# liuzuxin/FSRL

Hardware: NVIDIA H100
Metric: env-steps/sec (collect+update) SafetyCarCircle-v0 PPO-Lag (higher is better)
Workload: dtype f32

## Files before the change

### fsrl_b200/csrc/ppo_persist.cu

```cuda
#include "ppo_persist.cuh"
#include "arena.cuh"
#include "ppo_loss.cuh"
#include "wgmma.cuh"
#include <cuda_pipeline.h>
#include <cstdlib>
#include <cmath>
#include <vector>

namespace fsrl {
namespace pp {

using namespace wg;

constexpr int WQ = 2;
constexpr int NEPI = 128 * WQ;
constexpr int TPB = NEPI + 32;
constexpr int C1 = 16 / WQ;
constexpr int C2 = 32 / WQ;
constexpr int RB = 64;
constexpr int MB = 256;
constexpr int KC = 32, NCH = 256 / KC;
constexpr int SLOT_BYTES = 32768, NSLOT = 4;
constexpr int A_CHUNK = 64 * KC * 4;
constexpr int ACC_LD = 68;
constexpr int OUTP = 8;
constexpr int H_ = 256;
constexpr int IMG = 65536;
enum { I_H1A_HI, I_H1A_LO, I_H1T_HI, I_H1T_LO, I_DZA_HI, I_DZA_LO, I_DZT_HI, I_DZT_LO, I_W2A_HI, I_W2A_LO, I_W2B_HI, I_W2B_LO, N_IMG };
constexpr int DB2P_OFF = N_IMG * IMG;
constexpr int DW3P_OFF = DB2P_OFF + 4 * H_;
constexpr int DB3P_OFF = DW3P_OFF + 4 * H_ * OUTP;
constexpr int MAXD = 40;
constexpr int XS_OFF = 2 * SLOT_BYTES;
static_assert(XS_OFF >= 2 * 32 * 65 * 2 * 4 && XS_OFF >= 2 * (MAXD + 1) * 64 * 4 &&
              XS_OFF + 128 * (MAXD + 1) * 4 <= NSLOT * SLOT_BYTES, "staged rows overlap the ring's scratch or dW1 partials");
constexpr int NSMAX = (MAXD + 1) * 32 + 32 + 32 * OUTP + 16;
constexpr int SLICE_OFF = DB3P_OFF + 4 * 16;
constexpr int NET_WS = SLICE_OFF + 8 * NSMAX;
constexpr int SUMSQ_FLOATS = 128;
constexpr int FLAG_LINE = 32;
constexpr int F_A = 0, F_C = 1, F_PER_NET = 2;
constexpr int TILE_PK = (64 * 64 / NEPI + 2) / 3;
constexpr int TILE_FLOATS = TILE_PK * NEPI * 4;
constexpr int SLICE_PK = (NSMAX + 2) / 3;
constexpr int XG_PER_NET = 16 * TILE_FLOATS + 8 * SLICE_PK * 4;
constexpr int MAX_MB = 16384;
constexpr long long WAIT_CYCLES = 6000000000LL;

struct Args {
    fsrl_ppo_update_t u;
    int n_mb, slot0;
    long long adam_t0;
    float* ws;
    unsigned* flags;
    int* err;
    const float* adam_tab;
    long long* dbg;
    int dbg_step;
    unsigned dp_seq;
    int dp_direct;
};
constexpr int DBG_CH = 48;
constexpr int DBG_N = DBG_CH + 2 * 3 * NCH;
#define STAMP(i) do { if (P.dbg && t == P.dbg_step) P.dbg[(size_t)blockIdx.x * DBG_N + (i)] = clock64(); } while (0)

struct AdamS { float w1, b2, w2, rbc2s, eps, neg_step; };
__device__ __forceinline__ float adam_one(float p, float g, float& m, float& v, const AdamS& a) {
    m = m + a.w1 * (g - m);
    v = v * a.b2 + (a.w2 * g) * g;
    const float sq = v > 0.f ? v * rsqrtf(v) : 0.f;
    const float denom = fmaf(sq, a.rbc2s, a.eps);
    return p + __fdividef(a.neg_step * m, denom);
}

__device__ __forceinline__ void fail(int* err, int code) {
    *reinterpret_cast<volatile int*>(err) = code;
    __threadfence_system();
    asm volatile("trap;");
}
__device__ __forceinline__ uint32_t pk_hash(float x, float y, float z) {
    const uint32_t a = __float_as_uint(x), b = __float_as_uint(y), c = __float_as_uint(z);
    return a ^ __funnelshift_l(b, b, 11) ^ __funnelshift_l(c, c, 22);
}
__device__ __forceinline__ bool pk_ok(const float4& v, uint32_t tag) { return (__float_as_uint(v.w) ^ pk_hash(v.x, v.y, v.z)) == tag; }
__device__ __forceinline__ void st_packet(float* p, float x, float y, float z, uint32_t tag) {
    asm volatile("st.relaxed.sys.global.v4.f32 [%0], {%1,%2,%3,%4};" ::"l"(p), "f"(x), "f"(y), "f"(z), "f"(__uint_as_float(tag ^ pk_hash(x, y, z))) : "memory");
}
__device__ __forceinline__ float4 ld_packet(const float* p) {
    float4 v;
    asm volatile("ld.relaxed.sys.global.v4.f32 {%0,%1,%2,%3}, [%4];" : "=f"(v.x), "=f"(v.y), "=f"(v.z), "=f"(v.w) : "l"(p) : "memory");
    return v;
}

__device__ __noinline__ float3 dp_gather(const float* src, long long stride, int me, int world, uint32_t tag,
                                        float ox, float oy, float oz, int* err, int code) {
    const long long t0w = clock64();
    float ax = 0.f, ay = 0.f, az = 0.f;
    for (int r0 = 0; r0 < world; r0 += 4) {
        float4 v[4];
        bool ok;
        do {
            ok = true;
#pragma unroll
            for (int k = 0; k < 4; ++k)
                if (r0 + k < world && r0 + k != me) v[k] = ld_packet(src + (size_t)(r0 + k) * stride);
#pragma unroll
            for (int k = 0; k < 4; ++k)
                if (r0 + k < world && r0 + k != me) ok = ok && pk_ok(v[k], tag);
            if (!ok && clock64() - t0w > 4 * WAIT_CYCLES) fail(err, code);
        } while (!ok);
#pragma unroll
        for (int k = 0; k < 4; ++k) {
            if (r0 + k >= world) continue;
            if (r0 + k == me) { ax += ox; ay += oy; az += oz; }
            else { ax += v[k].x; ay += v[k].y; az += v[k].z; }
        }
    }
    return make_float3(ax, ay, az);
}
__device__ __noinline__ void dp_push_all(const float* const* xg, size_t off, int me, int world, float x, float y, float z, uint32_t tag) {
    for (int r = 0; r < world; ++r)
        if (r != me) st_packet(const_cast<float*>(xg[r]) + off, x, y, z, tag);
}

__device__ __forceinline__ uint32_t mapa_u32(uint32_t local_saddr, uint32_t rank) {
    uint32_t r;
    asm volatile("mapa.shared::cluster.u32 %0, %1, %2;" : "=r"(r) : "r"(local_saddr), "r"(rank));
    return r;
}
__device__ __forceinline__ void st_cluster4(uint32_t raddr, float4 v) {
    asm volatile("st.shared::cluster.v4.f32 [%0], {%1,%2,%3,%4};" ::"r"(raddr), "f"(v.x), "f"(v.y), "f"(v.z), "f"(v.w) : "memory");
}
__device__ __forceinline__ void st_async4(uint32_t raddr, float4 v, uint32_t rbar) {
    asm volatile("st.async.weak.shared::cluster.mbarrier::complete_tx::bytes.v4.f32 [%0], {%1,%2,%3,%4}, [%5];"
                 ::"r"(raddr), "f"(v.x), "f"(v.y), "f"(v.z), "f"(v.w), "r"(rbar) : "memory");
}
__device__ __forceinline__ float ld_cluster(uint32_t raddr) {
    float v;
    asm volatile("ld.shared::cluster.f32 %0, [%1];" : "=f"(v) : "r"(raddr) : "memory");
    return v;
}
__device__ __forceinline__ void mbar_arrive_release_cluster2(uint32_t raddr0, uint32_t raddr1) {
    asm volatile("fence.acq_rel.cluster;\n\t"
                 "mbarrier.arrive.relaxed.cluster.shared::cluster.b64 _, [%0];\n\t"
                 "mbarrier.arrive.relaxed.cluster.shared::cluster.b64 _, [%1];" ::"r"(raddr0), "r"(raddr1) : "memory");
}
__device__ __forceinline__ bool mbar_wait_cluster(uint64_t* bar, uint32_t parity, long long timeout_cycles) {
    const long long t0 = clock64();
    while (true) {
        uint32_t ok;
        asm volatile(
            "{\n\t.reg .pred p;\n\t"
            "mbarrier.try_wait.parity.acquire.cluster.shared::cta.b64 p, [%1], %2;\n\t"
            "selp.u32 %0, 1, 0, p;\n\t}"
            : "=r"(ok) : "r"(smem_u32(bar)), "r"(parity) : "memory");
        if (ok) return true;
        if (clock64() - t0 > timeout_cycles) return false;
    }
}
__device__ __forceinline__ void cluster_sync_all() {
    asm volatile("barrier.cluster.arrive.release.aligned;\n\tbarrier.cluster.wait.acquire.aligned;" ::: "memory");
}

__device__ __forceinline__ bool elect_one() {
    uint32_t pred = 0;
    asm volatile(
        "{\n\t.reg .b32 rx;\n\t.reg .pred px;\n\t"
        "elect.sync rx|px, 0xffffffff;\n\t"
        "selp.u32 %0, 1, 0, px;\n\t}"
        : "=r"(pred));
    return pred != 0;
}
__device__ __forceinline__ void epi_bar() { asm volatile("bar.sync 1, %0;" ::"n"(NEPI) : "memory"); }
__device__ __forceinline__ void prefetch_l2(const void* p) { asm volatile("prefetch.global.L2 [%0];" ::"l"(p)); }

template <int NC>
__device__ __forceinline__ void acc_ld(const float* accs, int row, int col, float (&v)[NC]) {
#pragma unroll
    for (int q = 0; q < NC / 4; ++q) {
        const float4 x = *reinterpret_cast<const float4*>(accs + row * ACC_LD + col + 4 * q);
        v[4 * q] = x.x; v[4 * q + 1] = x.y; v[4 * q + 2] = x.z; v[4 * q + 3] = x.w;
    }
}
template <int NC>
__device__ __forceinline__ void acc_st(float* accs, int row, int col, const float (&v)[NC]) {
#pragma unroll
    for (int q = 0; q < NC / 4; ++q)
        *reinterpret_cast<float4*>(accs + row * ACC_LD + col + 4 * q) = make_float4(v[4 * q], v[4 * q + 1], v[4 * q + 2], v[4 * q + 3]);
}

template <int N>
__device__ __forceinline__ void gemm_phase(const unsigned char* ring, unsigned& qq, uint64_t* bar_full, uint32_t empty_r,
                                           float (&dm)[N / 2], float (&dc)[N / 2], int* err, int code, int lane,
                                           const Args& P, int t, int g) {
#pragma unroll
    for (int e = 0; e < N / 2; ++e) dm[e] = dc[e] = 0.f;
    const uint32_t ring_a = smem_u32(ring);
    constexpr uint32_t b_lbo = 16 * N, b_chunk = N * KC * 4;
    for (int j = 0; j < NCH; ++j, ++qq) {
        const int s = qq % NSLOT;
        if (!mbar_wait(&bar_full[s], (qq / NSLOT) & 1, WAIT_CYCLES)) fail(err, code);
#ifdef FSRL_PPO_CHUNK_STAMPS
        if (P.dbg && t == P.dbg_step && threadIdx.x < 32) P.dbg[(size_t)blockIdx.x * DBG_N + DBG_CH + 3 * NCH * g + 2 * NCH + j] = clock64();
#endif
        __syncwarp();
        wgmma_fence();
        const uint32_t base = ring_a + (uint32_t)s * SLOT_BYTES;
        const uint64_t ah0 = smem_desc(base, 1024, 128), al0 = smem_desc(base + A_CHUNK, 1024, 128);
        const uint64_t bh0 = smem_desc(base + 2 * A_CHUNK, b_lbo, 128), bl0 = smem_desc(base + 2 * A_CHUNK + b_chunk, b_lbo, 128);
#pragma unroll
        for (int ks = 0; ks < KC / 8; ++ks) {
            const uint64_t ah = ah0 + ks * (2048 / 16), al = al0 + ks * (2048 / 16);
            const uint64_t bh = bh0 + ks * (2 * b_lbo / 16), bl = bl0 + ks * (2 * b_lbo / 16);
            if constexpr (N == 32) {
                mma_m64n32k8_tf32(dc, al, bh);
                mma_m64n32k8_tf32(dc, ah, bl);
                mma_m64n32k8_tf32(dm, ah, bh);
            } else {
                mma_m64n64k8_tf32(dc, al, bh);
                mma_m64n64k8_tf32(dc, ah, bl);
                mma_m64n64k8_tf32(dm, ah, bh);
            }
        }
        wgmma_commit();
        if (j > 0) {
            wgmma_wait<1>();
            __syncwarp();
            if (lane < 8) mbar_arrive_cluster(empty_r + 8 * ((qq - 1) % NSLOT));
        }
    }
    wgmma_wait<0>();
    reg_fence(dm); reg_fence(dc);
    __syncwarp();
    if (lane < 8) mbar_arrive_cluster(empty_r + 8 * ((qq - 1) % NSLOT));
}
template <int N>
__device__ __forceinline__ void stage_acc(float* accs, const float (&dm)[N / 2], const float (&dc)[N / 2], int wq, int sp,
                                          int lane) {
    if (wq == 0) {
        const int r = 16 * sp + (lane >> 2);
#pragma unroll
        for (int i = 0; i < N / 8; ++i) {
            const int c = 8 * i + 2 * (lane & 3);
            *reinterpret_cast<float2*>(accs + r * ACC_LD + c) = make_float2(dm[4 * i] + dc[4 * i], dm[4 * i + 1] + dc[4 * i + 1]);
            *reinterpret_cast<float2*>(accs + (r + 8) * ACC_LD + c) =
                make_float2(dm[4 * i + 2] + dc[4 * i + 2], dm[4 * i + 3] + dc[4 * i + 3]);
        }
    }
    asm volatile("bar.sync %0, 64;" ::"r"(2 + sp) : "memory");
}

__device__ __forceinline__ void copy_operand(unsigned char* dst, const float* src, uint32_t bytes, uint64_t* bar, int g, int i,
                                             uint16_t cta_mask) {
    if (g == 1) {
        bulk_g2s(dst, src, bytes, bar);
        bulk_g2s(dst + bytes, src + IMG, bytes, bar);
        return;
    }
    const uint32_t piece = 2 * bytes / g, off = i * piece, part = off / bytes, in = off % bytes;
    bulk_g2s_multicast(dst + off, src + (size_t)part * IMG + in / 4, piece, bar, cta_mask);
}

template <int NC, int W>
__device__ __forceinline__ void transposed_stage(float* scr, const float (&hi)[NC], const float (&lo)[NC], int row, int c0) {
    constexpr int LO = W * 65;
#pragma unroll
    for (int j = 0; j < NC; ++j) {
        scr[(c0 + j) * 65 + row] = hi[j];
        scr[LO + (c0 + j) * 65 + row] = lo[j];
    }
}
template <int W>
__device__ __forceinline__ void transposed_flush(const float* scr, int et, float* img_hi, int row_base, int col_base) {
    constexpr int LO = W * 65;
    const int col = et % W;
    constexpr int GPT = 16 / (NEPI / W);
    const int g0 = (et / W) * GPT;
    float* dst = img_hi + (size_t)(row_base >> 2) * 256 + (size_t)(col_base + col) * 4;
#pragma unroll
    for (int q = 0; q < GPT; ++q) {
        const int g = g0 + q;
        const float* sh = scr + col * 65 + 4 * g;
        *reinterpret_cast<float4*>(dst + (size_t)g * 256) = make_float4(sh[0], sh[1], sh[2], sh[3]);
        *reinterpret_cast<float4*>(dst + IMG + (size_t)g * 256) = make_float4(sh[LO], sh[LO + 1], sh[LO + 2], sh[LO + 3]);
    }
}
template <int NC, int W>
__device__ __forceinline__ void store_transposed(float* scr, const float (&hi)[NC], const float (&lo)[NC], int row, int c0,
                                                 int et, float* img_hi, int row_base, int col_base) {
    transposed_stage<NC, W>(scr, hi, lo, row, c0);
    epi_bar();
    transposed_flush<W>(scr, et, img_hi, row_base, col_base);
    epi_bar();
}

__device__ __forceinline__ void stage_rows(float* xs, const float* obs, long long row0, int a, int D, int et) {
    const int i = et >> 1;
    const float* src = obs + (row0 + 64 * a + i + (i & 64)) * D;
    float* dst = xs + i * (D | 1);
    for (int d = et & 1; d < D; d += 2) __pipeline_memcpy_async(dst + d, src + d, 4);
    __pipeline_commit();
}

__device__ __forceinline__ float half_sum(float v) {
#pragma unroll
    for (int o = 8; o > 0; o >>= 1) v += __shfl_xor_sync(0xffffffffu, v, o);
    return v;
}

struct SliceMap {
    int w1, b2, w3, b3, n;
    __device__ __host__ SliceMap(int D) { w1 = 0; b2 = (D + 1) * 32; w3 = b2 + 32; b3 = w3 + 32 * OUTP; n = b3 + 16; }
};

struct DpCtx {
    const float* const* xg;
    long long region;
    int me, world;
    uint32_t tag;
    int* err;
    int direct;
};
__device__ __forceinline__ int dp_owner(int et, int q, int world) { return (int)((unsigned)((et >> 5) * TILE_PK + q) % (unsigned)world); }

__device__ __noinline__ void dp_tile_send(DpCtx d, size_t off, const float* accs, int trow, int cb2, int et) {
    float g[C2];
    acc_ld<C2>(accs, trow, cb2, g);
#pragma unroll
    for (int q = 0; q < TILE_PK; ++q) {
        const size_t o_q = (size_t)d.me * d.region + off + (size_t)q * NEPI * 4;
        const float x = g[3 * q], y = 3 * q + 1 < C2 ? g[3 * q + 1] : 0.f, z = 3 * q + 2 < C2 ? g[3 * q + 2] : 0.f;
        if (d.direct) {
            dp_push_all(d.xg, o_q, d.me, d.world, x, y, z, d.tag);
        } else {
            const int o = dp_owner(et, q, d.world);
            if (o != d.me) st_packet(const_cast<float*>(d.xg[o]) + o_q, x, y, z, d.tag);
        }
    }
}
__device__ __noinline__ void dp_tile_reduce(DpCtx d, size_t off, float* accs, int trow, int cb2, int et) {
    float g[C2];
    acc_ld<C2>(accs, trow, cb2, g);
    const float inv_world = 1.0f / (float)d.world;
    const float* loc = d.xg[d.me];
#pragma unroll
    for (int q = 0; q < TILE_PK; ++q) {
        if (dp_owner(et, q, d.world) != d.me) continue;
        const float3 s3 = dp_gather(loc + off + (size_t)q * NEPI * 4, d.region, d.me, d.world, d.tag, g[3 * q],
                                    3 * q + 1 < C2 ? g[3 * q + 1] : 0.f, 3 * q + 2 < C2 ? g[3 * q + 2] : 0.f, d.err, 41);
        const float ax = s3.x * inv_world, ay = s3.y * inv_world, az = s3.z * inv_world;
        dp_push_all(d.xg, (size_t)FSRL_P2P_MAX_RANKS * d.region + off + (size_t)q * NEPI * 4, d.me, d.world, ax, ay, az, d.tag);
        g[3 * q] = ax;
        if (3 * q + 1 < C2) g[3 * q + 1] = ay;
        if (3 * q + 2 < C2) g[3 * q + 2] = az;
    }
    acc_st<C2>(accs, trow, cb2, g);
}
__device__ __noinline__ float dp_tile_finish(DpCtx d, size_t off, float* accs, int trow, int cb2, int et) {
    float g[C2];
    const long long t0w = clock64();
    if (d.direct) {
        float own[C2];
        acc_ld<C2>(accs, trow, cb2, own);
#pragma unroll
        for (int jq = 0; jq < C2; ++jq) g[jq] = 0.f;
        for (int r = 0; r < d.world; ++r) {
            if (r == d.me) {
#pragma unroll
                for (int jq = 0; jq < C2; ++jq) g[jq] += own[jq];
                continue;
            }
            const float* src = d.xg[d.me] + (size_t)r * d.region + off;
            float4 v[TILE_PK];
            bool ok;
            do {
                ok = true;
#pragma unroll
                for (int q = 0; q < TILE_PK; ++q) v[q] = ld_packet(src + (size_t)q * NEPI * 4);
#pragma unroll
                for (int q = 0; q < TILE_PK; ++q) ok = ok && pk_ok(v[q], d.tag);
                if (!ok && clock64() - t0w > 4 * WAIT_CYCLES) fail(d.err, 42);
            } while (!ok);
#pragma unroll
            for (int q = 0; q < TILE_PK; ++q) {
                g[3 * q] += v[q].x;
                if (3 * q + 1 < C2) g[3 * q + 1] += v[q].y;
                if (3 * q + 2 < C2) g[3 * q + 2] += v[q].z;
            }
        }
        const float inv_world = 1.0f / (float)d.world;
        float sq = 0.f;
#pragma unroll
        for (int jq = 0; jq < C2; ++jq) { g[jq] *= inv_world; sq = fmaf(g[jq], g[jq], sq); }
        acc_st<C2>(accs, trow, cb2, g);
        return sq;
    }
    const float* res = d.xg[d.me] + (size_t)FSRL_P2P_MAX_RANKS * d.region + off;
    acc_ld<C2>(accs, trow, cb2, g);
    float4 v[TILE_PK];
    bool ok;
    do {
        ok = true;
#pragma unroll
        for (int q = 0; q < TILE_PK; ++q)
            if (dp_owner(et, q, d.world) != d.me) v[q] = ld_packet(res + (size_t)q * NEPI * 4);
#pragma unroll
        for (int q = 0; q < TILE_PK; ++q)
            if (dp_owner(et, q, d.world) != d.me) ok = ok && pk_ok(v[q], d.tag);
        if (!ok && clock64() - t0w > 4 * WAIT_CYCLES) fail(d.err, 42);
    } while (!ok);
    float sq = 0.f;
#pragma unroll
    for (int q = 0; q < TILE_PK; ++q) {
        if (dp_owner(et, q, d.world) == d.me) continue;
        g[3 * q] = v[q].x;
        if (3 * q + 1 < C2) g[3 * q + 1] = v[q].y;
        if (3 * q + 2 < C2) g[3 * q + 2] = v[q].z;
    }
#pragma unroll
    for (int jq = 0; jq < C2; ++jq) sq = fmaf(g[jq], g[jq], sq);
    acc_st<C2>(accs, trow, cb2, g);
    return sq;
}
__device__ __noinline__ void dp_slices(DpCtx d, size_t off_s, float* sp_g, int n, int et) {
    const int n3 = (n + 2) / 3;
    const float inv_world = 1.0f / (float)d.world;
    for (int i = et; i < n3; i += NEPI)
        dp_push_all(d.xg, (size_t)d.me * d.region + off_s + 4 * (size_t)i, d.me, d.world,
                    sp_g[3 * i], 3 * i + 1 < n ? sp_g[3 * i + 1] : 0.f, 3 * i + 2 < n ? sp_g[3 * i + 2] : 0.f, d.tag);
    const float* loc = d.xg[d.me];
    for (int i = et; i < n3; i += NEPI) {
        const float3 s3 = dp_gather(loc + off_s + 4 * (size_t)i, d.region, d.me, d.world, d.tag, sp_g[3 * i],
                                    3 * i + 1 < n ? sp_g[3 * i + 1] : 0.f, 3 * i + 2 < n ? sp_g[3 * i + 2] : 0.f, d.err, 40);
        sp_g[3 * i] = s3.x * inv_world;
        if (3 * i + 1 < n) sp_g[3 * i + 1] = s3.y * inv_world;
        if (3 * i + 2 < n) sp_g[3 * i + 2] = s3.z * inv_world;
    }
}

__device__ __forceinline__ bool red_cta() { return ((blockIdx.x >> 3) & 3) == ((blockIdx.x & 7) >> 2); }

__device__ __noinline__ float dp_tail(DpCtx d, size_t off_t, size_t off_s, float* accs, float* sp_g, int n, int trow, int cb2,
                                      int et, bool tile, bool slice) {
    if (tile && !d.direct) dp_tile_reduce(d, off_t, accs, trow, cb2, et);
    if (slice) dp_slices(d, off_s, sp_g, n, et);
    __syncwarp();
    return tile ? dp_tile_finish(d, off_t, accs, trow, cb2, et) : 0.f;
}

template <bool DP>
__global__ void __launch_bounds__(TPB, 1) ppo_persist_kernel(const Args P) {
    extern __shared__ __align__(1024) unsigned char smem_raw[];
    __shared__ __align__(8) uint64_t bar_full[NSLOT], bar_empty[NSLOT], bar_b, bar_w1;
    __shared__ float s_red[4][320];
    __shared__ float s_misc[32];
    __shared__ AdamS s_adam;
    __shared__ const float* s_xg[2][FSRL_P2P_MAX_RANKS];
    const fsrl_ppo_update_t& u = P.u;
    const int tid = threadIdx.x, warp = tid >> 5, lane = tid & 31;
    const int net = blockIdx.x >> 5, c = blockIdx.x & 31, a = c >> 3, b = c & 7;
    const bool is_g2 = c < 16;
    const int ka = (c & 15) >> 2, q4 = c & 3;

    const int D = u.D, A = u.A, C = u.C, H = H_;
    const int out = (net == 0) ? A : 1;
    const int n_cta = 32 * u.n_nets;
    float* wsn = P.ws + (size_t)net * NET_WS;
    float* sumsq_g = P.ws + (size_t)u.n_nets * NET_WS;
    unsigned* fl_net = P.flags + (size_t)net * F_PER_NET * FLAG_LINE;
    unsigned* fl_d2 = P.flags + (size_t)u.n_nets * F_PER_NET * FLAG_LINE;
    unsigned char* ring = smem_raw;
    float* accs = reinterpret_cast<float*>(smem_raw + NSLOT * SLOT_BYTES);
    float* small = accs + 64 * ACC_LD;
    const SliceMap sm(D);
    float* sp_p = small;
    float* sp_m = small + sm.n;
    float* sp_v = small + 2 * sm.n;
    float* sp_g = small + 3 * sm.n;
    float* land = small + 4 * sm.n;

    if (tid == 0) {
        for (int i = 0; i < NSLOT; ++i) { mbar_init(&bar_full[i], 1); mbar_init(&bar_empty[i], 4 * 8); }
        mbar_init(&bar_b, 1);
        mbar_init(&bar_w1, 4);
        fence_mbar_init();
    }
    __syncthreads();
    if (DP && threadIdx.x < 2 * FSRL_P2P_MAX_RANKS) s_xg[threadIdx.x / FSRL_P2P_MAX_RANKS][threadIdx.x % FSRL_P2P_MAX_RANKS] = P.u.p2p_xg[threadIdx.x / FSRL_P2P_MAX_RANKS][threadIdx.x % FSRL_P2P_MAX_RANKS];
    if (DP) __syncthreads();
    cluster_sync_all();

    const long long pbase = u.net_off[net];
    const ArenaLayout L = arena_layout(D, H, out, 0);
    const long long o_w1 = pbase + L.w1, o_b1 = pbase + L.b1, o_w2 = pbase + L.w2, o_b2 = pbase + L.b2,
                    o_w3 = pbase + L.w3, o_b3 = pbase + L.b3, o_ls = pbase + L.extra;

    if (warp == NEPI / 32) {
        if (elect_one()) {
            unsigned qq = 0;
            for (int t = 0; t < P.n_mb; ++t) {
                if (!flag_wait_ge<true>(fl_net + F_A * FLAG_LINE, 32u * (t + 1), WAIT_CYCLES)) fail(P.err, 10);
                STAMP(12);
                fence_proxy_async_global();
#pragma unroll 1
                for (int j = 0; j < NCH; ++j, ++qq) {
                    const int s = qq % NSLOT;
                    if (!mbar_wait(&bar_empty[s], ((qq / NSLOT) & 1) ^ 1, WAIT_CYCLES)) fail(P.err, 11);
#ifdef FSRL_PPO_CHUNK_STAMPS
                    STAMP(DBG_CH + j);
#endif
                    unsigned char* dst = ring + (size_t)s * SLOT_BYTES;
                    mbar_expect_tx(&bar_full[s], 3 * A_CHUNK);
                    const size_t ao = (size_t)a * 16384 + (size_t)j * 64 * KC, bo = (size_t)b * 8192 + (size_t)j * 32 * KC;
                    copy_operand(dst, wsn + (size_t)I_H1A_HI * IMG + ao, A_CHUNK, &bar_full[s], 8, b, 0xff);
                    copy_operand(dst + 2 * A_CHUNK, wsn + (size_t)I_W2A_HI * IMG + bo, A_CHUNK / 2, &bar_full[s], 1, 0, 0);
#ifdef FSRL_PPO_CHUNK_STAMPS
                    STAMP(DBG_CH + NCH + j);
#endif
                }
                STAMP(13);
                if (!flag_wait_ge<true>(fl_net + F_C * FLAG_LINE, 32u * (t + 1), WAIT_CYCLES)) fail(P.err, 12);
                STAMP(14);
                fence_proxy_async_global();
                const int ia = is_g2 ? I_W2B_HI : I_DZT_HI, ib = is_g2 ? I_DZA_HI : I_H1T_HI;
                const int blk_a = is_g2 ? ka : q4, blk_b = is_g2 ? q4 : ka;
                const uint16_t m4 = (uint16_t)(0xfu << (b & 4)), m2 = (uint16_t)(0x11u << (b & 3));
#pragma unroll 1
                for (int j = 0; j < NCH; ++j, ++qq) {
                    const int s = qq % NSLOT;
                    if (!mbar_wait(&bar_empty[s], ((qq / NSLOT) & 1) ^ 1, WAIT_CYCLES)) fail(P.err, 13);
#ifdef FSRL_PPO_CHUNK_STAMPS
                    STAMP(DBG_CH + 3 * NCH + j);
#endif
                    unsigned char* dst = ring + (size_t)s * SLOT_BYTES;
                    mbar_expect_tx(&bar_full[s], 4 * A_CHUNK);
                    const size_t ao = (size_t)blk_a * 16384 + (size_t)j * 64 * KC, bo = (size_t)blk_b * 16384 + (size_t)j * 64 * KC;
                    copy_operand(dst, wsn + (size_t)ia * IMG + ao, A_CHUNK, &bar_full[s], is_g2 ? 4 : 2, is_g2 ? b & 3 : b >> 2, is_g2 ? m4 : m2);
                    copy_operand(dst + 2 * A_CHUNK, wsn + (size_t)ib * IMG + bo, A_CHUNK, &bar_full[s], is_g2 ? 2 : 4, is_g2 ? b >> 2 : b & 3, is_g2 ? m2 : m4);
#ifdef FSRL_PPO_CHUNK_STAMPS
                    STAMP(DBG_CH + 4 * NCH + j);
#endif
                }
            }
        }
    } else {
        const int et = tid;
        const int sp = warp & 3;
        const int wq = warp >> 2;
        const int r16 = lane & 15, half = lane >> 4;
        const int trow = 16 * sp + r16;
        const int cb1 = 16 * half + C1 * wq;
        const int cb2 = 32 * half + C2 * wq;
        unsigned qq = 0;
        const uint32_t empty_r = mapa_u32(smem_u32(bar_empty), lane < 8 ? lane : 0);
        float w2p[C2], w2m[C2], w2v[C2];
        const int world = DP ? u.world : 1;
        auto dp_ctx = [&](int t_) {
            DpCtx d;
            const unsigned long long id = (unsigned long long)(P.adam_t0 + t_ + 1);
            d.xg = s_xg[(int)(id & 1ULL)];
            d.region = (long long)u.n_nets * XG_PER_NET;
            d.me = u.p2p_rank; d.world = world;
            d.tag = (P.dp_seq << 16) | (uint32_t)((t_ + 1) & 0xffff);
            d.err = P.err;
            d.direct = P.dp_direct;
            return d;
        };

        float* xs = reinterpret_cast<float*>(ring + XS_OFF);
        if (is_g2) stage_rows(xs, u.obs, 0, a, D, et);
        for (int i = et; i < sm.n; i += NEPI) {
            long long src = -1;
            if (i < sm.b2) { const int d = i / 32, kk = i % 32; src = (d < D) ? o_w1 + (long long)d * H + 32 * b + kk : o_b1 + 32 * b + kk; }
            else if (i < sm.w3) src = o_b2 + 32 * b + (i - sm.b2);
            else if (i < sm.b3) { const int oo = (i - sm.w3) / OUTP, jj = (i - sm.w3) % OUTP; if (jj < out) src = o_w3 + (long long)(32 * b + oo) * out + jj; }
            else { const int jj = i - sm.b3; if (jj < out) src = o_b3 + jj; else if (net == 0 && jj >= 8 && jj < 8 + A) src = o_ls + (jj - 8); }
            sp_p[i] = src >= 0 ? u.theta[src] : 0.f;
            sp_m[i] = src >= 0 ? u.adam_m[src] : 0.f;
            sp_v[i] = src >= 0 ? u.adam_v[src] : 0.f;
            sp_g[i] = 0.f;
        }
        if (!is_g2) {
            const int o = 64 * q4 + trow;
#pragma unroll
            for (int j = 0; j < C2; ++j) {
                const long long idx = o_w2 + (long long)(64 * ka + cb2 + j) * H + o;
                w2p[j] = u.theta[idx]; w2m[j] = u.adam_m[idx]; w2v[j] = u.adam_v[idx];
            }
        } else {
#pragma unroll
            for (int j = 0; j < C2; ++j) w2p[j] = w2m[j] = w2v[j] = 0.f;
        }
        __pipeline_wait_prior(0);
        epi_bar();

        for (int t = 0; t < P.n_mb; ++t) {
            const long long row0 = (long long)t * MB;
            const int slot = P.slot0 + t;
            if (et == 0) {
                s_adam.w1 = (float)(1.0 - u.beta1); s_adam.b2 = (float)u.beta2; s_adam.w2 = (float)(1.0 - u.beta2);
                s_adam.rbc2s = __ldg(P.adam_tab + 2 * t); s_adam.eps = (float)u.adam_eps; s_adam.neg_step = __ldg(P.adam_tab + 2 * t + 1);
                STAMP(0);
                if (P.dbg && t == P.dbg_step) { long long gt; asm volatile("mov.u64 %0, %%globaltimer;" : "=l"(gt)); P.dbg[(size_t)blockIdx.x * DBG_N + 30] = gt; }
                if (P.dbg && t == P.dbg_step + 64) {
                    long long gt; asm volatile("mov.u64 %0, %%globaltimer;" : "=l"(gt));
                    P.dbg[(size_t)blockIdx.x * DBG_N + 31] = gt;
                    P.dbg[(size_t)blockIdx.x * DBG_N + 29] = clock64();
                }
            }
            if (t + 1 < P.n_mb && et < 64) {
                const long long r = row0 + MB + 64 * a + et;
                prefetch_l2(u.obs + r * D);
                if (D > 32) prefetch_l2(u.obs + r * D + 32);
                if (is_g2) { prefetch_l2(u.obs + (r + 128) * D); if (D > 32) prefetch_l2(u.obs + (r + 128) * D + 32); }
                if (net == 0) { prefetch_l2(u.act + r * A); prefetch_l2(u.logp_old + r); prefetch_l2(u.adv + r); if (C > 1) prefetch_l2(u.adv + u.ld + r); }
                else { prefetch_l2(u.ret + (long long)(net - 1) * u.ld + r); if (u.value_clip) prefetch_l2(u.values + (long long)(net - 1) * u.ld + r); }
            }
            float* scratch = reinterpret_cast<float*>(ring);
            if (!is_g2) {
                const float (&pv)[C2] = w2p;
                float phi[C2], plo[C2];
                const int o = 64 * q4 + trow;
                float* w2a_hi = wsn + (size_t)I_W2A_HI * IMG + (size_t)(o >> 5) * 8192 + (size_t)(o & 31) * 4;
                float* w2a_lo = w2a_hi + IMG;
#pragma unroll
                for (int q = 0; q < C2 / 4; ++q) {
                    float4 hi, lo;
                    tf32_split(pv[4 * q], hi.x, lo.x); tf32_split(pv[4 * q + 1], hi.y, lo.y);
                    tf32_split(pv[4 * q + 2], hi.z, lo.z); tf32_split(pv[4 * q + 3], hi.w, lo.w);
                    const size_t plane = (size_t)(16 * ka + (cb2 >> 2) + q) * 128;
                    *reinterpret_cast<float4*>(w2a_hi + plane) = hi;
                    *reinterpret_cast<float4*>(w2a_lo + plane) = lo;
                    phi[4 * q] = hi.x; phi[4 * q + 1] = hi.y; phi[4 * q + 2] = hi.z; phi[4 * q + 3] = hi.w;
                    plo[4 * q] = lo.x; plo[4 * q + 1] = lo.y; plo[4 * q + 2] = lo.z; plo[4 * q + 3] = lo.w;
                }
                store_transposed<C2, 64>(scratch, phi, plo, trow, cb2, et, wsn + (size_t)I_W2B_HI * IMG + (size_t)ka * 16384, 64 * q4, 0);
            }
            if (is_g2) {
                const int r = et & 63, kc = C1 * (et >> 6);
                const float* x0 = xs + r * (D | 1);
                const float* x1 = xs + (64 + r) * (D | 1);
                float acc2[2][C1];
#pragma unroll
                for (int j = 0; j < C1; ++j) acc2[0][j] = acc2[1][j] = sp_p[sm.w1 + D * 32 + kc + j];
                for (int d = 0; d < D; ++d) {
                    const float xv0 = x0[d], xv1 = x1[d];
                    const float* w = sp_p + sm.w1 + d * 32 + kc;
#pragma unroll
                    for (int j = 0; j < C1; ++j) { acc2[0][j] = fmaf(xv0, w[j], acc2[0][j]); acc2[1][j] = fmaf(xv1, w[j], acc2[1][j]); }
                }
                constexpr int TSCR = 2 * 32 * 65;
#pragma unroll
                for (int rep = 0; rep < 2; ++rep) {
                    const int aa = a + 2 * rep;
                    float hi[C1], lo[C1];
                    float* a_hi = wsn + (size_t)I_H1A_HI * IMG + (size_t)aa * 16384 + (size_t)r * 4;
#pragma unroll
                    for (int q = 0; q < C1 / 4; ++q) {
#pragma unroll
                        for (int e = 0; e < 4; ++e) tf32_split(fmaxf(acc2[rep][4 * q + e], 0.f), hi[4 * q + e], lo[4 * q + e]);
                        const size_t plane = (size_t)(8 * b + (kc >> 2) + q) * 256;
                        *reinterpret_cast<float4*>(a_hi + plane) = make_float4(hi[4 * q], hi[4 * q + 1], hi[4 * q + 2], hi[4 * q + 3]);
                        *reinterpret_cast<float4*>(a_hi + IMG + plane) = make_float4(lo[4 * q], lo[4 * q + 1], lo[4 * q + 2], lo[4 * q + 3]);
                    }
                    transposed_stage<C1, 32>(scratch + rep * TSCR, hi, lo, r, kc);
                }
                epi_bar();
#pragma unroll
                for (int rep = 0; rep < 2; ++rep)
                    transposed_flush<32>(scratch + rep * TSCR, et, wsn + (size_t)I_H1T_HI * IMG + (size_t)(b >> 1) * 16384, 64 * (a + 2 * rep), 32 * (b & 1));
            }
            fence_proxy_async_smem();
            epi_bar();
            if (et == 0) { STAMP(1); flag_add_release(fl_net + F_A * FLAG_LINE); }

            const long long grow = row0 + 64 * a + trow;
            float p_act[8], p_lpo = 0.f, p_adv0 = 0.f, p_adv1 = 0.f, p_ret = 0.f, p_val = 0.f, mean[2] = {0.f, 0.f}, rstd[2] = {1.f, 1.f};
#pragma unroll
            for (int j = 0; j < 8; ++j) p_act[j] = 0.f;
            if (net == 0) {
#pragma unroll
                for (int j = 0; j < 8; ++j) if (j < A) p_act[j] = __ldg(u.act + grow * A + j);
                p_lpo = __ldg(u.logp_old + grow);
                p_adv0 = __ldg(u.adv + grow);
                if (C > 1) p_adv1 = __ldg(u.adv + u.ld + grow);
                const float* ms = u.mb_stats + (size_t)t * 4;
                mean[0] = __ldg(ms); rstd[0] = __ldg(ms + 1); mean[1] = __ldg(ms + 2); rstd[1] = __ldg(ms + 3);
            } else {
                p_ret = __ldg(u.ret + (long long)(net - 1) * u.ld + grow);
                if (u.value_clip) p_val = __ldg(u.values + (long long)(net - 1) * u.ld + grow);
            }
            float p_ls[8], p_rsg[8];
#pragma unroll
            for (int j = 0; j < 8; ++j) {
                p_ls[j] = (net == 0 && j < A) ? sp_p[sm.b3 + 8 + j] : 0.f;
                p_rsg[j] = 1.0f / expf(p_ls[j]);
            }

            {
                float dm[16], dc[16];
                if (wq == 0) gemm_phase<32>(ring, qq, bar_full, empty_r, dm, dc, P.err, 30, lane, P, t, 0);
                else qq += NCH;
                stage_acc<32>(accs, dm, dc, wq, sp, lane);
            }
            if (et == 0) STAMP(2);
            float h2[C1];
            acc_ld<C1>(accs, trow, cb1, h2);
            float hp[OUTP];
#pragma unroll
            for (int j = 0; j < OUTP; ++j) hp[j] = 0.f;
#pragma unroll
            for (int j = 0; j < C1; ++j) {
                h2[j] = fmaxf(h2[j] + sp_p[sm.b2 + cb1 + j], 0.f);
                const float* w = sp_p + sm.w3 + (cb1 + j) * OUTP;
#pragma unroll
                for (int jj = 0; jj < OUTP; ++jj) hp[jj] = fmaf(h2[j], w[jj], hp[jj]);
            }
#pragma unroll
            for (int jj = 0; jj < OUTP; ++jj) hp[jj] += __shfl_xor_sync(0xffffffffu, hp[jj], 16);
            if (WQ > 1) {
                float* xh = &s_red[0][0];
                if (half == 0 && wq > 0) {
#pragma unroll
                    for (int jj = 0; jj < OUTP; ++jj) xh[((wq - 1) * 64 + trow) * OUTP + jj] = hp[jj];
                }
                epi_bar();
                if (half == 0 && wq == 0) {
#pragma unroll
                    for (int w2 = 1; w2 < WQ; ++w2)
#pragma unroll
                        for (int jj = 0; jj < OUTP; ++jj) hp[jj] += xh[((w2 - 1) * 64 + trow) * OUTP + jj];
                }
            }
            float outv[OUTP];
#pragma unroll
            for (int jj = 0; jj < OUTP; ++jj) outv[jj] = sp_p[sm.b3 + jj];
            if (et == 0) {
                STAMP(3);
                mbar_expect_tx(&bar_b, 8u * 64u * OUTP * (uint32_t)sizeof(float));
            }
            if (half == 0 && wq == 0) {
                const uint32_t mine = smem_u32(land + ((size_t)b * 64 + trow) * OUTP);
                const uint32_t bb_ = smem_u32(&bar_b);
#pragma unroll
                for (int r = 0; r < 8; ++r) {
                    const uint32_t ra = mapa_u32(mine, r), rb = mapa_u32(bb_, r);
                    st_async4(ra, make_float4(hp[0], hp[1], hp[2], hp[3]), rb);
                    st_async4(ra + 16, make_float4(hp[4], hp[5], hp[6], hp[7]), rb);
                }
            }
            if (!mbar_wait_cluster(&bar_b, t & 1, WAIT_CYCLES)) fail(P.err, 31);
            __syncwarp();
            if (et == 0) STAMP(4);
#pragma unroll
            for (int bb = 0; bb < 8; ++bb) {
                const float* src = land + ((size_t)bb * 64 + trow) * OUTP;
                const float4 v0 = *reinterpret_cast<const float4*>(src);
                const float4 v1 = *reinterpret_cast<const float4*>(src + 4);
                outv[0] += v0.x; outv[1] += v0.y; outv[2] += v0.z; outv[3] += v0.w;
                outv[4] += v1.x; outv[5] += v1.y; outv[6] += v1.z; outv[7] += v1.w;
            }
            float dd[16];
#pragma unroll
            for (int j = 0; j < 16; ++j) dd[j] = 0.f;
            float st_a = 0.f, st_b = 0.f, st_c = 0.f, st_d = 0.f;
            {
                const float invB = 1.0f / (float)MB;
                if (net == 0) {
                    float g_mu[8], g_ls[8];
                    ppo_actor_row(u, outv, p_act, p_ls, p_rsg, p_lpo, p_adv0, p_adv1, mean, rstd, invB, g_mu, g_ls,
                                  st_a, st_b, st_c);
#pragma unroll
                    for (int j = 0; j < 8; ++j) { dd[j] = g_mu[j]; dd[8 + j] = g_ls[j]; }
                } else {
                    dd[0] = ppo_value_row(u, outv[0], p_ret, p_val, invB, st_d);
                }
            }
            if (et == 0) STAMP(26);
            const int nfeed = (net == 0) ? A : 1;
            float dz[C1];
#pragma unroll
            for (int j = 0; j < C1; ++j) {
                const float* w = sp_p + sm.w3 + (cb1 + j) * OUTP;
                float g = 0.f;
#pragma unroll
                for (int jj = 0; jj < OUTP; ++jj) if (jj < nfeed) g = fmaf(dd[jj], w[jj], g);
                dz[j] = h2[j] > 0.f ? g : 0.f;
            }
            {
                float hi[C1], lo[C1];
                float* a_hi = wsn + (size_t)I_DZA_HI * IMG + (size_t)a * 16384 + (size_t)trow * 4;
#pragma unroll
                for (int q = 0; q < C1 / 4; ++q) {
#pragma unroll
                    for (int e = 0; e < 4; ++e) tf32_split(dz[4 * q + e], hi[4 * q + e], lo[4 * q + e]);
                    const size_t plane = (size_t)(8 * b + (cb1 >> 2) + q) * 256;
                    *reinterpret_cast<float4*>(a_hi + plane) = make_float4(hi[4 * q], hi[4 * q + 1], hi[4 * q + 2], hi[4 * q + 3]);
                    *reinterpret_cast<float4*>(a_hi + IMG + plane) = make_float4(lo[4 * q], lo[4 * q + 1], lo[4 * q + 2], lo[4 * q + 3]);
                }
                store_transposed<C1, 32>(scratch, hi, lo, trow, cb1, et, wsn + (size_t)I_DZT_HI * IMG + (size_t)(b >> 1) * 16384, 64 * a, 32 * (b & 1));
            }
            if (et == 0) STAMP(27);
            {
                float* row = &s_red[sp][0];
#pragma unroll
                for (int j = 0; j < C1; ++j) {
                    const float sdz = half_sum(dz[j]);
                    if (r16 == 0) row[cb1 + j] = sdz;
                }
#pragma unroll
                for (int jj = 0; jj < OUTP; ++jj) {
                    if (jj < nfeed) {
#pragma unroll
                        for (int j = 0; j < C1; ++j) {
                            const float sv = half_sum(h2[j] * dd[jj]);
                            if (r16 == 0) row[32 + 32 * jj + cb1 + j] = sv;
                        }
                    }
                }
                if (b == 0 && wq == 0) {
#pragma unroll
                    for (int j = 0; j < 16; ++j) {
                        const float sv = half_sum(dd[j]);
                        if (lane == 0) row[288 + j] = sv;
                    }
                    const float sa = half_sum(st_a), sb = half_sum(st_b), sc = half_sum(st_c), sdv = half_sum(st_d);
                    if (lane == 0) { row[304] = sa; row[305] = sb; row[306] = sc; row[307] = sdv; }
                }
            }
            epi_bar();
            if (et == 0) STAMP(28);
            for (int i = et; i < 32 + 32 * nfeed; i += NEPI) {
                const float tot = ((s_red[0][i] + s_red[1][i]) + s_red[2][i]) + s_red[3][i];
                if (i < 32) wsn[DB2P_OFF + a * H + 32 * b + i] = tot;
                else wsn[DW3P_OFF + ((size_t)a * H + 32 * b + ((i - 32) & 31)) * OUTP + ((i - 32) >> 5)] = tot;
            }
            if (b == 0) {
                if (et < 20) {
                    const int i = 288 + et;
                    const float tot = ((s_red[0][i] + s_red[1][i]) + s_red[2][i]) + s_red[3][i];
                    if (et < 16) wsn[DB3P_OFF + a * 16 + et] = tot;
                    else {
                        float* stat = u.stats + (size_t)slot * FSRL_PPO_STATS;
                        if (net == 0) { if (et == 16) atomicAdd(stat + ST_ACTOR_REW, tot); if (et == 17) atomicAdd(stat + ST_ACTOR_SAFETY, tot); if (et == 18) atomicAdd(stat + ST_KL, tot); }
                        else if (et == 19) atomicAdd(stat + ST_VF0 + (net - 1), tot);
                    }
                }
                if (net == 0 && a == 0 && et == 20) u.stats[(size_t)slot * FSRL_PPO_STATS + ST_ENTROPY] = ppo_entropy(sp_p + sm.b3 + 8, A);
            }
            fence_proxy_async_smem();
            epi_bar();
            if (et == 0) { STAMP(5); flag_add_release(fl_net + F_C * FLAG_LINE); }

            unsigned mbits = 0;
            if (is_g2) {
                const int k = 64 * ka + trow;
                const float* msk = wsn + (size_t)I_H1A_HI * IMG + (size_t)q4 * 16384 + (size_t)(k >> 2) * 256 + (k & 3);
                float mreg[C2];
#pragma unroll
                for (int jq = 0; jq < C2; ++jq) mreg[jq] = __ldcg(msk + (size_t)(cb2 + jq) * 4);
                float xr[(64 * MAXD + NEPI - 1) / NEPI];
                const int nx = (64 * D + NEPI - 1) / NEPI;
                const float* xb = u.obs + (row0 + 64 * q4) * D;
#pragma unroll
                for (int q = 0; q < (64 * MAXD + NEPI - 1) / NEPI; ++q)
                    xr[q] = (q < nx && et + q * NEPI < 64 * D) ? __ldg(xb + et + q * NEPI) : 0.f;
#pragma unroll
                for (int jq = 0; jq < C2; ++jq) mbits |= (mreg[jq] > 0.f ? 1u : 0u) << jq;
#pragma unroll
                for (int q = 0; q < (64 * MAXD + NEPI - 1) / NEPI; ++q) {
                    const int e = et + q * NEPI;
                    if (q < nx && e < 64 * D) { const int r = e / D; land[r * ((D + 3) & ~3) + 4 * (r >> 5) + (e - r * D)] = xr[q]; }
                }
            }
            if (red_cta() && wq == 1) {
                const int tw = et - 128;
                if (tw == 0) {
                    if (!flag_wait_ge(fl_net + F_C * FLAG_LINE, 32u * (t + 1), WAIT_CYCLES)) fail(P.err, 35);
                    STAMP(15);
                }
                asm volatile("bar.sync 6, 128;" ::: "memory");
                for (int i0 = sm.b2 + tw; i0 < sm.n; i0 += 4 * 128) {
                    float pv[4][4];
#pragma unroll
                    for (int e = 0; e < 4; ++e) {
                        const int i = i0 + e * 128;
                        const float* src = wsn;
                        size_t stride = 0;
                        bool real = false;
                        if (i < sm.n) {
                            if (i < sm.w3) { src = wsn + DB2P_OFF + 32 * b + (i - sm.b2); stride = H; real = true; }
                            else if (i < sm.b3) {
                                const int oo = (i - sm.w3) / OUTP, jj = (i - sm.w3) % OUTP;
                                real = jj < out;
                                src = wsn + DW3P_OFF + ((size_t)32 * b + oo) * OUTP + jj; stride = (size_t)H * OUTP;
                            } else {
                                const int jj = i - sm.b3;
                                real = (jj < out) || (net == 0 && jj >= 8 && jj < 8 + A);
                                src = wsn + DB3P_OFF + jj; stride = 16;
                            }
                        }
#pragma unroll
                        for (int q = 0; q < 4; ++q) pv[e][q] = real ? __ldcg(src + q * stride) : 0.f;
                    }
#pragma unroll
                    for (int e = 0; e < 4; ++e) {
                        const int i = i0 + e * 128;
                        if (i < sm.n) {
                            float gsum = 0.f;
#pragma unroll
                            for (int q = 0; q < 4; ++q) gsum += pv[e][q];
                            sp_g[i] = gsum;
                        }
                    }
                }
                if (tw == 0) STAMP(16);
            }
            {
                float dm[32], dc[32];
                if (wq == 0) gemm_phase<64>(ring, qq, bar_full, empty_r, dm, dc, P.err, 32, lane, P, t, 1);
                else qq += NCH;
                stage_acc<64>(accs, dm, dc, wq, sp, lane);
            }
            if (et == 0) STAMP(6);
            float sq = 0.f;
            if (is_g2) {
                float v[C2];
                acc_ld<C2>(accs, trow, cb2, v);
#pragma unroll
                for (int jq = 0; jq < C2; ++jq) v[jq] = ((mbits >> jq) & 1u) ? v[jq] : 0.f;
                epi_bar();
                if (et == 0) STAMP(22);
                const int dp4 = (D + 3) & ~3;
                const float* xh = land + (size_t)cb2 * dp4 + 4 * half;
                float* dst = reinterpret_cast<float*>(ring) + (size_t)wq * (D + 1) * 64 + trow;
                for (int d0 = 0; d0 < D; d0 += 4) {
                    float sacc[4] = {0.f, 0.f, 0.f, 0.f};
#pragma unroll
                    for (int jq = 0; jq < C2; ++jq) {
                        const float4 x = *reinterpret_cast<const float4*>(xh + jq * dp4 + d0);
                        sacc[0] = fmaf(x.x, v[jq], sacc[0]);
                        sacc[1] = fmaf(x.y, v[jq], sacc[1]);
                        sacc[2] = fmaf(x.z, v[jq], sacc[2]);
                        sacc[3] = fmaf(x.w, v[jq], sacc[3]);
                    }
#pragma unroll
                    for (int i = 0; i < 4; ++i) sacc[i] += __shfl_xor_sync(0xffffffffu, sacc[i], 16);
                    if (half == 0) {
#pragma unroll
                        for (int i = 0; i < 4; ++i)
                            if (d0 + i < D) dst[(d0 + i) * 64] = sacc[i];
                    }
                }
                float sb1 = 0.f;
#pragma unroll
                for (int jq = 0; jq < C2; ++jq) sb1 += v[jq];
                sb1 += __shfl_xor_sync(0xffffffffu, sb1, 16);
                if (half == 0) dst[D * 64] = sb1;
                if (et == 0) STAMP(23);
                epi_bar();
                if (et == 0) mbar_arrive_release_cluster2(mapa_u32(smem_u32(&bar_w1), 2 * ka), mapa_u32(smem_u32(&bar_w1), 2 * ka + 1));
            } else {
                float g[C2];
                acc_ld<C2>(accs, trow, cb2, g);
                if (DP) {
                    dp_tile_send(dp_ctx(t), (size_t)(net * 16 + (c - 16)) * TILE_FLOATS + (size_t)et * 4, accs, trow, cb2, et);
                    if (et == 0) STAMP(32);
                } else {
#pragma unroll
                    for (int jq = 0; jq < C2; ++jq) sq = fmaf(g[jq], g[jq], sq);
                }
            }
            if (et == 0) STAMP(7);
            if (red_cta()) {
                if (!mbar_wait_cluster(&bar_w1, t & 1, WAIT_CYCLES)) fail(P.err, 33);
                if (et == 0) STAMP(8);
                const uint32_t ring_s = smem_u32(ring);
                const int kb = 32 * (b & 1);
                for (int i0 = et; i0 < sm.b2; i0 += 2 * NEPI) {
                    float pv[2][4 * WQ];
#pragma unroll
                    for (int e = 0; e < 2; ++e) {
                        const int i = i0 + e * NEPI;
                        const uint32_t off = 4u * (uint32_t)((i / 32) * 64 + kb + (i % 32));
#pragma unroll
                        for (int rb = 0; rb < 4; ++rb) {
                            const uint32_t src = mapa_u32(ring_s + off, (uint32_t)((4 * (b >> 1) + rb) & 7));
#pragma unroll
                            for (int w = 0; w < WQ; ++w)
                                pv[e][WQ * rb + w] = i < sm.b2 ? ld_cluster(src + 4u * (uint32_t)(w * (D + 1) * 64)) : 0.f;
                        }
                    }
#pragma unroll
                    for (int e = 0; e < 2; ++e) {
                        const int i = i0 + e * NEPI;
                        if (i < sm.b2) {
                            float gsum = 0.f;
#pragma unroll
                            for (int q = 0; q < 4 * WQ; ++q) gsum += pv[e][q];
                            sp_g[i] = gsum;
                        }
                    }
                }
                epi_bar();
                if (et == 0) STAMP(17);
            }
            if (DP) {
                const DpCtx d = dp_ctx(t);
                const size_t off_t = (size_t)(net * 16 + (c - 16)) * TILE_FLOATS + (size_t)et * 4;
                sq += dp_tail(d, off_t, (size_t)u.n_nets * 16 * TILE_FLOATS + (size_t)(net * 8 + b) * SLICE_PK * 4, accs, sp_g, sm.n,
                              trow, cb2, et, !is_g2, red_cta());
                if (et == 0) STAMP(41);
                epi_bar();
            }
            if (red_cta()) {
                for (int i = et; i < sm.n; i += NEPI) {
                    bool real = true;
                    if (i >= sm.w3 && i < sm.b3) real = ((i - sm.w3) % OUTP) < out;
                    else if (i >= sm.b3) { const int jj = i - sm.b3; real = (jj < out) || (net == 0 && jj >= 8 && jj < 8 + A); }
                    if (real && (i < sm.b3 || b == 0)) sq = fmaf(sp_g[i], sp_g[i], sq);
                    wsn[SLICE_OFF + (size_t)b * NSMAX + i] = sp_g[i];
                }
            }
            if (red_cta() || !is_g2) {
                sq = warp_sum(sq);
                if (lane == 0) s_misc[warp] = sq;
                epi_bar();
                if (et == 0) {
                    float tot = 0.f;
#pragma unroll
                    for (int w2 = 0; w2 < NEPI / 32; ++w2) tot += s_misc[w2];
                    sumsq_g[blockIdx.x - (red_cta() ? 8 * a : 0)] = tot;
                    STAMP(9);
                    flag_add_release(fl_d2);
                }
            }
            if (is_g2 && t + 1 < P.n_mb) stage_rows(xs, u.obs, row0 + MB, a, D, et);
            if (et == 0) {
                if (!flag_wait_ge(fl_d2, 24u * (unsigned)u.n_nets * (t + 1), WAIT_CYCLES)) fail(P.err, 34);
                STAMP(10);
            }
            epi_bar();
            float nq[4];
#pragma unroll
            for (int q = 0; q < 4; ++q) nq[q] = (lane + 32 * q < n_cta) ? __ldcg(sumsq_g + lane + 32 * q) : 0.f;
            if (!DP && !red_cta())
                for (int i = et; i < sm.n; i += NEPI) sp_g[i] = __ldcg(wsn + SLICE_OFF + (size_t)b * NSMAX + i);
            float nsq = ((nq[0] + nq[1]) + nq[2]) + nq[3];
            nsq = warp_sum(nsq);
            float gscale = 1.0f;
            if (u.max_grad_norm > 0.f) gscale = fminf(u.max_grad_norm / (sqrtf(nsq) + 1e-6f), 1.0f);
            if (blockIdx.x == 0 && et == 0) u.stats[(size_t)slot * FSRL_PPO_STATS + ST_GRADNORM] = sqrtf(nsq);
            const AdamS ad = s_adam;
            if (et == 0) STAMP(24);
            for (int i = et; i < sm.n; i += NEPI) {
                float m = sp_m[i], v = sp_v[i];
                const float g = (DP && !red_cta()) ? __ldcg(wsn + SLICE_OFF + (size_t)b * NSMAX + i) : sp_g[i];
                sp_p[i] = adam_one(sp_p[i], g * gscale, m, v, ad);
                sp_m[i] = m; sp_v[i] = v;
            }
            if (et == 0) STAMP(25);
            if (!is_g2) {
                float g[C2];
                acc_ld<C2>(accs, trow, cb2, g);
#pragma unroll
                for (int j = 0; j < C2; ++j) w2p[j] = adam_one(w2p[j], g[j] * gscale, w2m[j], w2v[j], ad);
            } else {
                __pipeline_wait_prior(0);
                if (et == 0) STAMP(18);
            }
            epi_bar();
            if (et == 0) STAMP(11);
        }

        if (a == 0) {
            for (int i = et; i < sm.n; i += NEPI) {
                long long dst = -1;
                if (i < sm.b2) { const int d = i / 32, kk = i % 32; dst = (d < D) ? o_w1 + (long long)d * H + 32 * b + kk : o_b1 + 32 * b + kk; }
                else if (i < sm.w3) dst = o_b2 + 32 * b + (i - sm.b2);
                else if (i < sm.b3) { const int oo = (i - sm.w3) / OUTP, jj = (i - sm.w3) % OUTP; if (jj < out) dst = o_w3 + (long long)(32 * b + oo) * out + jj; }
                else if (b == 0) { const int jj = i - sm.b3; if (jj < out) dst = o_b3 + jj; else if (net == 0 && jj >= 8 && jj < 8 + A) dst = o_ls + (jj - 8); }
                if (dst >= 0) { u.theta[dst] = sp_p[i]; u.adam_m[dst] = sp_m[i]; u.adam_v[dst] = sp_v[i]; }
            }
        }
        if (!is_g2) {
            const int o = 64 * q4 + trow;
#pragma unroll
            for (int j = 0; j < C2; ++j) {
                const long long idx = o_w2 + (long long)(64 * ka + cb2 + j) * H + o;
                u.theta[idx] = w2p[j]; u.adam_m[idx] = w2m[j]; u.adam_v[idx] = w2v[j];
            }
        }
    }
    __syncthreads();
    cluster_sync_all();
}

static size_t smem_bytes(int D) {
    return (size_t)NSLOT * SLOT_BYTES + sizeof(float) * 64 * ACC_LD + 4 * sizeof(float) * SliceMap(D).n +
           sizeof(float) * 8 * 64 * OUTP;
}

static cudaLaunchConfig_t cluster_launch(int n_nets, size_t smem, cudaStream_t s, cudaLaunchAttribute* at) {
    at->id = cudaLaunchAttributeClusterDimension;
    at->val.clusterDim.x = 8; at->val.clusterDim.y = 1; at->val.clusterDim.z = 1;
    cudaLaunchConfig_t cfg = {};
    cfg.gridDim = dim3(32 * n_nets); cfg.blockDim = dim3(TPB); cfg.dynamicSmemBytes = smem; cfg.stream = s;
    cfg.attrs = at; cfg.numAttrs = 1;
    return cfg;
}

struct Instance {
    void (*kern)(const Args);
    int max_clusters;
};
static const Instance& instance(bool dp) {
    static Instance inst[2] = {};
    Instance& in = inst[dp];
    if (!in.kern) {
        in.kern = dp ? ppo_persist_kernel<true> : ppo_persist_kernel<false>;
        cudaLaunchAttribute at;
        const cudaLaunchConfig_t cfg = cluster_launch(1, smem_bytes(MAXD), nullptr, &at);
        if (cudaFuncSetAttribute(in.kern, cudaFuncAttributeMaxDynamicSharedMemorySize, (int)cfg.dynamicSmemBytes) != cudaSuccess ||
            cudaOccupancyMaxActiveClusters(&in.max_clusters, in.kern, &cfg) != cudaSuccess) {
            cudaGetLastError();
            in.max_clusters = 0;
        }
    }
    return in;
}

}

size_t ppo_persist_ws_floats(int n_nets, int D, int H) {
    (void)D; (void)H;
    return (size_t)n_nets * pp::NET_WS + pp::SUMSQ_FLOATS + (size_t)(n_nets * pp::F_PER_NET + 1) * pp::FLAG_LINE + 32 +
           2 * (size_t)pp::MAX_MB + 2 * (size_t)32 * n_nets * pp::DBG_N;
}

size_t ppo_persist_p2p_floats(int n_nets) { return (size_t)(FSRL_P2P_MAX_RANKS + 1) * n_nets * pp::XG_PER_NET + 64; }

bool ppo_persist_supported(const fsrl_ppo_update_t& u, long long n_total, int batch_size) {
    if (u.H != 256 || batch_size != pp::MB || n_total % pp::MB != 0 || n_total < pp::MB || n_total / pp::MB > pp::MAX_MB) return false;
    if (u.world > 1 && !(u.p2p_on && u.world <= FSRL_P2P_MAX_RANKS && (size_t)u.p2p_stride >= ppo_persist_p2p_floats(u.n_nets))) return false;
    if (u.D < 1 || u.D > pp::MAXD || u.A > 8 || u.n_nets < 1 || u.n_nets > 3) return false;
    if (u.persist_ws == nullptr || (size_t)u.persist_ws_floats < ppo_persist_ws_floats(u.n_nets, u.D, u.H)) return false;
    if (32 * u.n_nets > sm_count()) return false;
    return pp::instance(u.world > 1).max_clusters >= 4 * u.n_nets;
}

int ppo_persist_run(const fsrl_ppo_update_t& ug, int n_mb, int stats_slot0, long long adam_t0, cudaStream_t s) {
    pp::Args a;
    a.u = ug;
    a.n_mb = n_mb; a.slot0 = stats_slot0; a.adam_t0 = adam_t0;
    a.ws = ug.persist_ws;
    const size_t fl_off = (size_t)ug.n_nets * pp::NET_WS + pp::SUMSQ_FLOATS;
    a.flags = reinterpret_cast<unsigned*>(ug.persist_ws + fl_off);
    const size_t n_flag_words = (size_t)(ug.n_nets * pp::F_PER_NET + 1) * pp::FLAG_LINE;
    a.err = reinterpret_cast<int*>(a.flags + n_flag_words);
    FSRL_CUDA(cudaMemsetAsync(ug.persist_ws + fl_off - pp::SUMSQ_FLOATS, 0, (pp::SUMSQ_FLOATS + n_flag_words + 32) * sizeof(float), s));
    float* tab_dev = reinterpret_cast<float*>(a.err + 32);
    static std::vector<float> tab;
    tab.resize(2 * (size_t)n_mb);
    for (int t = 0; t < n_mb; ++t) {
        const double tt = (double)(adam_t0 + t + 1);
        const double bc1 = 1.0 - pow(ug.beta1, tt), bc2 = 1.0 - pow(ug.beta2, tt);
        tab[2 * t] = (float)(1.0 / sqrt(bc2));
        tab[2 * t + 1] = (float)(-(ug.lr / bc1));
    }
    FSRL_CUDA(cudaMemcpyAsync(tab_dev, tab.data(), tab.size() * sizeof(float), cudaMemcpyHostToDevice, s));
    a.adam_tab = tab_dev;
    static unsigned dp_seq = 0;
    if (ug.world > 1) dp_seq = (dp_seq % 65535u) + 1u;
    a.dp_seq = dp_seq;
    a.dp_direct = ug.world <= 2;
    if (const char* e = getenv("FSRL_PPO_DP_DIRECT")) a.dp_direct = atoi(e) != 0;
    a.dbg = nullptr; a.dbg_step = -1;
    if (const char* e = getenv("FSRL_PPO_PERSIST_DBG")) {
        a.dbg = reinterpret_cast<long long*>(tab_dev + 2 * (size_t)pp::MAX_MB);
        a.dbg_step = atoi(e);
    }
    cudaLaunchAttribute at;
    const cudaLaunchConfig_t cfg = pp::cluster_launch(ug.n_nets, pp::smem_bytes(ug.D), s, &at);
    FSRL_CUDA(cudaLaunchKernelEx(&cfg, pp::instance(ug.world > 1).kern, a));
    ++g_launches;
    return FSRL_OK;
}

}
```

Measured before the change: 3.017 million.

## Defer transposed H1/W2 image stores past the flag release into accumulator scratch

Moves the transposed hi/lo staging and flush of the H1 activations and W2 images from before the F_A flag release to after it, so the consumer network can start on the row-major images sooner. Staging now goes through the accumulator tile (accs) instead of the ring scratch, with a new static_assert that the staging buffer fits there. The W2 transpose is split into two 32-column halves. In exchange the tf32 split is recomputed, acc2 stays live across the barrier (more register pressure), and extra epilogue barriers are added.

After: 2.985 million (median of 6 runs). 0.99x the previous value.

```diff
diff --git a/fsrl_b200/csrc/ppo_persist.cu b/fsrl_b200/csrc/ppo_persist.cu
--- a/fsrl_b200/csrc/ppo_persist.cu
+++ b/fsrl_b200/csrc/ppo_persist.cu
@@ -32,8 +32,9 @@
 constexpr int DB3P_OFF = DW3P_OFF + 4 * H_ * OUTP;
 constexpr int MAXD = 40;
 constexpr int XS_OFF = 2 * SLOT_BYTES;
-static_assert(XS_OFF >= 2 * 32 * 65 * 2 * 4 && XS_OFF >= 2 * (MAXD + 1) * 64 * 4 &&
-              XS_OFF + 128 * (MAXD + 1) * 4 <= NSLOT * SLOT_BYTES, "staged rows overlap the ring's scratch or dW1 partials");
+static_assert(XS_OFF >= 2 * (MAXD + 1) * 64 * 4 &&
+              XS_OFF + 128 * (MAXD + 1) * 4 <= NSLOT * SLOT_BYTES, "staged rows overlap the dW1 partials");
+static_assert(2 * 32 * 65 <= 64 * ACC_LD, "a [64 x 32] hi / lo transpose staging does not fit the accumulator tile");
 constexpr int NSMAX = (MAXD + 1) * 32 + 32 + 32 * OUTP + 16;
 constexpr int SLICE_OFF = DB3P_OFF + 4 * 16;
 constexpr int NET_WS = SLICE_OFF + 8 * NSMAX;
@@ -619,7 +620,6 @@
             float* scratch = reinterpret_cast<float*>(ring);
             if (!is_g2) {
                 const float (&pv)[C2] = w2p;
-                float phi[C2], plo[C2];
                 const int o = 64 * q4 + trow;
                 float* w2a_hi = wsn + (size_t)I_W2A_HI * IMG + (size_t)(o >> 5) * 8192 + (size_t)(o & 31) * 4;
                 float* w2a_lo = w2a_hi + IMG;
@@ -631,16 +631,13 @@
                     const size_t plane = (size_t)(16 * ka + (cb2 >> 2) + q) * 128;
                     *reinterpret_cast<float4*>(w2a_hi + plane) = hi;
                     *reinterpret_cast<float4*>(w2a_lo + plane) = lo;
-                    phi[4 * q] = hi.x; phi[4 * q + 1] = hi.y; phi[4 * q + 2] = hi.z; phi[4 * q + 3] = hi.w;
-                    plo[4 * q] = lo.x; plo[4 * q + 1] = lo.y; plo[4 * q + 2] = lo.z; plo[4 * q + 3] = lo.w;
-                }
-                store_transposed<C2, 64>(scratch, phi, plo, trow, cb2, et, wsn + (size_t)I_W2B_HI * IMG + (size_t)ka * 16384, 64 * q4, 0);
-            }
+                }
+            }
+            float acc2[2][C1];
             if (is_g2) {
                 const int r = et & 63, kc = C1 * (et >> 6);
                 const float* x0 = xs + r * (D | 1);
                 const float* x1 = xs + (64 + r) * (D | 1);
-                float acc2[2][C1];
 #pragma unroll
                 for (int j = 0; j < C1; ++j) acc2[0][j] = acc2[1][j] = sp_p[sm.w1 + D * 32 + kc + j];
                 for (int d = 0; d < D; ++d) {
@@ -649,7 +646,6 @@
 #pragma unroll
                     for (int j = 0; j < C1; ++j) { acc2[0][j] = fmaf(xv0, w[j], acc2[0][j]); acc2[1][j] = fmaf(xv1, w[j], acc2[1][j]); }
                 }
-                constexpr int TSCR = 2 * 32 * 65;
 #pragma unroll
                 for (int rep = 0; rep < 2; ++rep) {
                     const int aa = a + 2 * rep;
@@ -663,16 +659,37 @@
                         *reinterpret_cast<float4*>(a_hi + plane) = make_float4(hi[4 * q], hi[4 * q + 1], hi[4 * q + 2], hi[4 * q + 3]);
                         *reinterpret_cast<float4*>(a_hi + IMG + plane) = make_float4(lo[4 * q], lo[4 * q + 1], lo[4 * q + 2], lo[4 * q + 3]);
                     }
-                    transposed_stage<C1, 32>(scratch + rep * TSCR, hi, lo, r, kc);
-                }
-                epi_bar();
-#pragma unroll
-                for (int rep = 0; rep < 2; ++rep)
-                    transposed_flush<32>(scratch + rep * TSCR, et, wsn + (size_t)I_H1T_HI * IMG + (size_t)(b >> 1) * 16384, 64 * (a + 2 * rep), 32 * (b & 1));
+                }
             }
             fence_proxy_async_smem();
             epi_bar();
             if (et == 0) { STAMP(1); flag_add_release(fl_net + F_A * FLAG_LINE); }
+            if (is_g2) {
+                const int r = et & 63, kc = C1 * (et >> 6);
+#pragma unroll
+                for (int rep = 0; rep < 2; ++rep) {
+                    float hi[C1], lo[C1];
+#pragma unroll
+                    for (int j = 0; j < C1; ++j) tf32_split(fmaxf(acc2[rep][j], 0.f), hi[j], lo[j]);
+                    transposed_stage<C1, 32>(accs, hi, lo, r, kc);
+                    epi_bar();
+                    transposed_flush<32>(accs, et, wsn + (size_t)I_H1T_HI * IMG + (size_t)(b >> 1) * 16384, 64 * (a + 2 * rep), 32 * (b & 1));
+                    epi_bar();
+                }
+            } else {
+#pragma unroll
+                for (int p = 0; p < 2; ++p) {
+                    if (half == p) {
+                        float hi[C2], lo[C2];
+#pragma unroll
+                        for (int j = 0; j < C2; ++j) tf32_split(w2p[j], hi[j], lo[j]);
+                        transposed_stage<C2, 32>(accs, hi, lo, trow, cb2 - 32 * p);
+                    }
+                    epi_bar();
+                    transposed_flush<32>(accs, et, wsn + (size_t)I_W2B_HI * IMG + (size_t)ka * 16384, 64 * q4, 32 * p);
+                    epi_bar();
+                }
+            }
 
             const long long grow = row0 + 64 * a + trow;
             float p_act[8], p_lpo = 0.f, p_adv0 = 0.f, p_adv1 = 0.f, p_ret = 0.f, p_val = 0.f, mean[2] = {0.f, 0.f}, rstd[2] = {1.f, 1.f};
```
